# zhan994/agi_lidar_slam

Measured on AMD Instinct MI355X. Metric: IKF iterations/sec, 100k-pt scan vs 10M-pt map, higher is better.
Workload: dtype f32 (kNN, plane) + f64 (Jacobian, reduction, 24x24 update); 1 GPU; C2: S-FAST_LIO update_iterated_dyn_share_modified, 100000-pt Avia scan vs 10000000-pt map, 4 IKF iterations per step with the 5-NN search every iteration; map_points=10000000, scan_points=100000, control_flow=fixed, maximum_iter=4, ikf_loop=device-resident, parallelism=single GPU, effective_points=91373

## Files before the change

### agi_lidar_slam_amd/csrc/slio_device.hip

```cpp
#include <hip/hip_ext.h>
#include <hip/hip_runtime.h>
#include <hipcub/hipcub.hpp>
#include <rccl/rccl.h>

#include <algorithm>
#include <type_traits>
#include <atomic>
#include <cmath>
#include <cstdlib>
#include <cstdio>
#include <cstddef>
#include <cstring>
#include <type_traits>
#include <memory>
#include <mutex>
#include <shared_mutex>
#include <string>
#include <vector>

#include "slio_common.hpp"
#include "slio_cvsolve.hpp"
#include "slio_device.hpp"
#include "slio_frontend.h"
#include "slio_plane.hpp"
// ... 1689 lines not shown
      row[12] = -(double)pd2;
      row[13] = 1.0;
    }
    st_out(out.sel + i, (uint8_t)(sel ? 1 : 0));
  }
  st_out(out.resid + i, sel ? pd2 : __int_as_float(0x7fc00000));
}

__device__ __forceinline__ double chunk_sums_256(double (*rows)[kRow], double (*part)[SLIO_NPROD],
                                                 bool mfma) {
  return mfma ? chunk_products_mfma_v<256>(rows) : chunk_products_v<256>(rows, part);
}

template <bool SC1>
__device__ __forceinline__ void ikf_dx_new(IkfCtl* ctl) {
  if (blockIdx.x != 0) return;
  const int t = threadIdx.x;
  auto ld = [](const double* p) { return SC1 ? ld_sc1(p) : *p; };
  if (t < 24) {
    const int k = t;
    if (k < 3 || k >= 9) {
      const double* xs = reinterpret_cast<const double*>(&ctl->x);
      const double* ps = reinterpret_cast<const double*>(&ctl->xprop);
      st_sc1(&ctl->dxn[k], ld(xs + state_off(k)) - ld(ps + state_off(k)));
    }
  } else if (t == 32 || t == 64) {
    const int u = t == 32;
    const double* q1 = u ? ctl->x.rli : ctl->x.rot;
    const double* q2 = u ? ctl->xprop.rli : ctl->xprop.rot;
    double d[3];
    so3_boxminus(Quat{ld(q1), ld(q1 + 1), ld(q1 + 2), ld(q1 + 3)}, Quat{ld(q2), ld(q2 + 1), ld(q2 + 2), ld(q2 + 3)},
                 d);
    st_sc1(&ctl->dxn[3 + 3 * u], d[0]);
    st_sc1(&ctl->dxn[4 + 3 * u], d[1]);
    st_sc1(&ctl->dxn[5 + 3 * u], d[2]);
  }
}

struct FuseArgs {
  IkfCtl* ctl;
  const IkfCtl* pre;
  double* seg_out;
  double* super_out;
  const IkfCtl* src;
  IkfCtl* hblk;
  uint32_t* cnt;
  double R;
  int iter, maxit;
  int64_t C;
  int nrows, s0, granks;
  double* gsup;
  uint32_t* garrive;
  int32_t gseq;
  uint64_t* goflag;
  uint64_t wait_ticks;
};
constexpr int kGoFlagStride = 16;
constexpr int kSegCnt = 16;
constexpr int kCountWords = kSegCnt + kNSeg;
constexpr int kKcCount = 8;

__device__ __forceinline__ int seg_of_chunk(int64_t C, int64_t c, int64_t& lim) {
  int s = 0;
#pragma unroll
  for (int q = 1; q < SLIO_NSUPER; ++q) s = super_lo(C, q) <= c ? q : s;
  const int64_t c0 = super_lo(C, s), c1 = super_lo(C, s + 1);
  const int g = (int)((c - c0) % kSuperSeg);
  lim = (c1 - c0 - g + kSuperSeg - 1) / kSuperSeg;
  return s * kSuperSeg + g;
}

template <int D>
__device__ __forceinline__ void prefetch_ctl(const IkfCtl* __restrict__ hsrc, IkfCtl* __restrict__ ctl) {
  constexpr int nC = CtlList<D>::total;
  const double* hs = reinterpret_cast<const double*>(hsrc);
  double* cd = reinterpret_cast<double*>(ctl);
  for (int e = threadIdx.x; e < nC; e += blockDim.x) {
    const int o = ctl_src<D>(e);
    st_sc1(cd + o, ld_sys(hs + o));
  }
  if (threadIdx.x < 8)
    st_sc1_u32(reinterpret_cast<uint32_t*>(&ctl->converge) + threadIdx.x,
               ld_sys_u32(reinterpret_cast<const uint32_t*>(&hsrc->converge) + threadIdx.x));
  if (threadIdx.x == 8) st_sc1_u32(reinterpret_cast<uint32_t*>(&ctl->singular), 0u);
  if (threadIdx.x == 9)
    st_sc1_u32(reinterpret_cast<uint32_t*>(&ctl->seq), ld_sys_u32(reinterpret_cast<const uint32_t*>(&hsrc->seq)));
}

template <int NT, int D, bool WT = false>
__device__ __forceinline__ void fused_tail(StepLds& L, int& bcast, const FuseArgs& fa, IkfCtl* ctl,
                                           const double* chunk_part, int64_t chunk, int iter) {
  const int t = threadIdx.x;
  int64_t lim;
  const int b = seg_of_chunk(fa.C, chunk, lim);
#ifdef SLIO_SOLVE_STAMP
  unsigned long long ts[4] = {0, 0, 0, 0};
  if (t == 0) ts[0] = wall_clock64();
#endif
  drain_stores();
  __syncthreads();
  if (t == 0) bcast = (int)arrive(fa.cnt + kSegCnt + b);
  __syncthreads();
#ifdef SLIO_SOLVE_STAMP
  if (t == 0) ts[1] = wall_clock64();
#endif
  if (bcast != (int)lim - 1) return;
  if (t < SLIO_NPROD) {
    const int s = b / kSuperSeg, g = b - s * kSuperSeg;
    const double* p = chunk_part + (super_lo(fa.C, s) + g) * SLIO_NPROD + t;
    constexpr int kJ = 16;
    double acc = 0.0;
    for (int64_t j0 = 0; j0 < lim; j0 += kJ) {
      double v[kJ];
#pragma unroll
      for (int j = 0; j < kJ; ++j) v[j] = (j0 + j < lim) ? ld_sc1(p + (j0 + j) * (kSuperSeg * SLIO_NPROD)) : 0.0;
#pragma unroll
      for (int j = 0; j < kJ; ++j) acc = acc + v[j];
    }
    st_sc1(fa.seg_out + b * SLIO_NPROD + t, acc);
  }
  if (t == 0) reset_counter(fa.cnt + kSegCnt + b);
  drain_stores();
  __syncthreads();
#ifdef SLIO_SOLVE_STAMP
  if (t == 0) ts[2] = wall_clock64();
#endif
  if (t == 0) bcast = (int)arrive(fa.cnt);
  __syncthreads();
  if (bcast != fa.nrows - 1) return;
#ifdef SLIO_SOLVE_STAMP
  if (t == 0) {
    ts[3] = wall_clock64();
    for (int k = 0; k < 4; ++k) g_sstamp[16 + k] = ts[k];
    g_sstamp[36 + ((iter + 1) & 3)] = ts[0];
    g_sstamp[32 + ((iter + 1) & 3)] = ts[3];
  }
#endif
  if (t == 0) {
    reset_counter(fa.cnt);
    st_sc1_u32(fa.cnt + 6, ld_sc1_u32(fa.cnt + 5));
    st_sc1_u32(fa.cnt + 4, 0u);
    st_sc1_u32(fa.cnt + 5, 0u);
  }
  if (!fa.gsup) {
    final_step<NT, D, true, false, WT>(L, fa.seg_out, fa.super_out, ctl, fa.src, fa.hblk, fa.R, iter, fa.maxit);
    if (WT && fa.goflag) {
      drain_stores();
      __syncthreads();
      if (t < 8) {
        const uint64_t fl = ((uint64_t)(uint32_t)fa.gseq << 32) | (L.fl[F_DONE] ? 0x80000000ull : 0ull) |
                            (uint64_t)(uint32_t)L.fl[F_PASSES];
        __hip_atomic_store((guint64*)(fa.goflag + t * kGoFlagStride), fl, __ATOMIC_RELAXED,
                           __HIP_MEMORY_SCOPE_AGENT);
      }
    }
  } else {
    const int nsup = SLIO_NSUPER / fa.granks;
    if (t < SLIO_NPROD) {
      for (int k = 0; k < nsup; ++k) {
        const int ss = fa.s0 + k;
        double a = ld_sc1(fa.seg_out + (ss * kSuperSeg) * SLIO_NPROD + t);
#pragma unroll
        for (int q = 1; q < kSuperSeg; ++q) a = a + ld_sc1(fa.seg_out + (ss * kSuperSeg + q) * SLIO_NPROD + t);
        st_sc1(fa.gsup + ss * SLIO_NPROD + t, a);
      }
      if (!fa.garrive)
        for (int ss = 0; ss < SLIO_NSUPER; ++ss)
          if (ss < fa.s0 || ss >= fa.s0 + nsup) st_sc1(fa.gsup + ss * SLIO_NPROD + t, 0.0);
    }
    if (!fa.garrive) return;
    drain_stores();
    __syncthreads();
    if (t == 0) bcast = (int)arrive(fa.garrive);
    __syncthreads();
    if (bcast != fa.granks - 1) return;
    if (t == 0) reset_counter(fa.garrive);
    final_step<NT, D, true, true>(L, fa.gsup, nullptr, ctl, fa.src, fa.hblk, fa.R, iter, fa.maxit);
    drain_stores();
    __syncthreads();
    if (t == 0) {
      __builtin_amdgcn_fence(__ATOMIC_RELEASE, "agent");
      asm volatile("s_waitcnt vmcnt(0)" ::: "memory");
      const uint64_t fl = ((uint64_t)(uint32_t)fa.gseq << 32) | (L.fl[F_DONE] ? 0x80000000ull : 0ull) |
                          (uint64_t)(uint32_t)L.fl[F_PASSES];
      __hip_atomic_store((guint64*)(uint64_t*)(fa.garrive + 2), fl, __ATOMIC_RELAXED, __HIP_MEMORY_SCOPE_AGENT);
    }
  }
#ifdef SLIO_SOLVE_STAMP
  if (t == 0) g_sstamp[25 + ((iter + 1) & 3)] = wall_clock64();
#endif
}

#ifndef SLIO_RL8_MAX
#define SLIO_RL8_MAX 8
#endif
struct RefLds {
  uint64_t top[SLIO_CHUNK][5];
  float4 q[SLIO_CHUNK];
  uint8_t slot[SLIO_CHUNK];
};
template <int NT>
struct SearchLds {
  union {
    double rows[SLIO_CHUNK][kRow];
    RefLds ref;
  } rr;
  double part[NT / 128][SLIO_NPROD];
  alignas(16) uint32_t nb_pos[SLIO_CHUNK][5];
  alignas(16) float nb_sqd[SLIO_CHUNK][5];
  alignas(16) int32_t nb_idx[SLIO_CHUNK][5];
  float nb_d5[SLIO_CHUNK];
  float4 qw[SLIO_CHUNK];
  float4 qb[SLIO_CHUNK];
  float4 qpl[SLIO_CHUNK];
  uint32_t kc_n[2];
  uint32_t kx6[SLIO_CHUNK];
  uint8_t ksame[SLIO_CHUNK];
  int far_cnt, ref_cnt;
  uint32_t cost;
  uint32_t tab_pre[NT / 16][kTab];
  int32_t tab_dl[NT / 16][kTab];
  float4 far_q[SLIO_CHUNK];
  uint8_t far_slot[SLIO_CHUNK];
  uint32_t far_pre[NT / 64][64], far_beg[NT / 64][64];
};
template <int NT>
union PassLds {
  SearchLds<NT> s;
  StepLds L;
};

template <int LPQ, int U, bool SPHERE, bool DEVPOSE, bool FUSE, int FD, bool PERS>
__device__ __forceinline__ void search_pass_body(PassLds<search_block<LPQ>()>& lds, int& fuse_bcast,
                                                 const MapView& map, const ScanDev& scan, const PoseDev& pose,
                                                 const PassCfg& cfg, const PassOut& out, const FuseArgs& fa,
                                                 bool reuse, int iter) {
  constexpr int NT = search_block<LPQ>();
  constexpr bool KC = DEVPOSE && LPQ == 2 && !SPHERE;
  if (DEVPOSE) ikf_dx_new<PERS>(cfg.ctl);
  constexpr int QPP = NT / LPQ;
  constexpr int PASSES = SLIO_CHUNK / QPP;
  static_assert(SLIO_CHUNK % QPP == 0, "chunk must be a multiple of queries/pass");
  static_assert(NT >= SLIO_CHUNK, "fit phase needs one lane per point");
  auto& rows = lds.s.rr.rows;
  auto& ref = lds.s.rr.ref;
  auto& part = lds.s.part;
  auto& nb_pos = lds.s.nb_pos;
  auto& nb_sqd = lds.s.nb_sqd;
  auto& nb_idx = lds.s.nb_idx;
  auto& nb_d5 = lds.s.nb_d5;
  auto& qw = lds.s.qw;
  auto& far_cnt = lds.s.far_cnt;
  auto& ref_cnt = lds.s.ref_cnt;
  auto& tab_pre = lds.s.tab_pre;
  auto& tab_dl = lds.s.tab_dl;
  auto& far_q = lds.s.far_q;
  auto& far_slot = lds.s.far_slot;
  auto& far_pre = lds.s.far_pre;
  auto& far_beg = lds.s.far_beg;
  int64_t chunk = xcd_chunk(cfg.c_begin, cfg.c_end - cfg.c_begin);
  const int tid = threadIdx.x;
  if (reuse) {
    if (tid < SLIO_CHUNK) {
      double row[kRow];
      reuse_row(scan, pose, cfg, out, chunk * SLIO_CHUNK + tid, row);
#pragma unroll
      for (int j = 0; j < kRow; ++j) lds.s.rr.rows[tid][j] = row[j];
    }
    __syncthreads();
  } else {
  if (cfg.perm) {
    const uint32_t pc = cfg.perm[chunk - cfg.c_begin];
    if (pc < (uint32_t)(cfg.c_end - cfg.c_begin)) chunk = cfg.c_begin + pc;
  }
  const int sub = tid & (LPQ - 1);
  const int grp = tid / LPQ;
  const GridGeom g = map.g;
  const float4* __restrict__ pts = map.pts;
  const uint32_t* __restrict__ start = map.start;
  bool cache_ok = false;
  if constexpr (KC) {
    const uint32_t ke = PERS ? __builtin_amdgcn_readfirstlane(ld_sc1_u32(&out.kepoch[chunk])) : out.kepoch[chunk];
    cache_ok = cfg.kc_epoch != 0 && ke == cfg.kc_epoch;
  }
  if (tid == 0) STAMP(0);
  if (tid == 0) {
    far_cnt = 0;
    ref_cnt = 0;
    lds.s.cost = 0;
    if (KC) lds.s.kc_n[0] = lds.s.kc_n[1] = 0;
    if (blockIdx.x == 0 && !cfg.knn_only) *out.pose = pose;
  }
// ... 407 lines not shown
      }
    }
    FSTAMP(3, false);
#pragma unroll
    for (int j = 0; j < kRow; ++j) rows[slot][j] = row[j];
    FSTAMP(4, true);
  }
  __syncthreads();
  if (tid == 0) STAMP(2);
  if (tid == 0 && out.chunk_cost)
    out.chunk_cost[chunk - cfg.c_begin] = lds.s.cost + 256u * (uint32_t)ref_cnt + 1024u * (uint32_t)nfar;
  if constexpr (KC) {
    if (tid == 0 && cfg.kc_epoch) {
      if (!cache_ok) out.kepoch[chunk] = cfg.kc_epoch;
      if (out.kc_count) {
        atomicAdd(out.kc_count, lds.s.kc_n[0]);
        atomicAdd(out.kc_count + 1, lds.s.kc_n[1]);
      }
    }
  }
  {
    const int64_t base = chunk * SLIO_CHUNK;
    const int nw = (int)(5 * min((int64_t)SLIO_CHUNK, scan.n - base));
    const int na = cfg.knn_only ? 3 : 1;
    auto dst = [&](int a) {
      return a == 0 ? out.nbr_pos + base * 5
                    : (uint32_t*)(a == 1 ? (void*)out.nbr_idx : (void*)out.nbr_sqd) + base * 5;
    };
    auto src = [&](int a) {
      return a == 0 ? &nb_pos[0][0]
                    : (const uint32_t*)(a == 1 ? (const void*)&nb_idx[0][0] : (const void*)&nb_sqd[0][0]);
    };
    if ((nw & 3) == 0) {
      const int nv = nw >> 2;
      for (int k = tid; k < na * nv; k += NT) {
        const int a = k >= nv ? (k >= 2 * nv ? 2 : 1) : 0;
        const int v = k - a * nv;
        st_out(reinterpret_cast<uint4*>(dst(a)) + v, reinterpret_cast<const uint4*>(src(a))[v]);
      }
    } else {
      for (int k = tid; k < na * nw; k += NT) {
        const int a = k >= nw ? (k >= 2 * nw ? 2 : 1) : 0;
        const int v = k - a * nw;
        st_out(dst(a) + v, src(a)[v]);
      }
    }
  }
  }
  if (cfg.knn_only) return;
  if constexpr (FUSE) {
    const double pv = chunk_sums_256(rows, part, cfg.mfma);
    if (tid < SLIO_NPROD) st_sc1(out.chunk_part + chunk * SLIO_NPROD + tid, pv);
    if (tid == 0) STAMP(3);
    fused_tail<NT, FD, PERS>(lds.L, fuse_bcast, fa, fa.ctl, out.chunk_part, chunk, iter);
  } else {
    if constexpr (NT == 256) {
      const double pv = chunk_sums_256(rows, part, cfg.mfma);
      if (tid < SLIO_NPROD) out.chunk_part[chunk * SLIO_NPROD + tid] = pv;
    } else {
      chunk_products<NT>(rows, part, out.chunk_part + chunk * SLIO_NPROD);
    }
    if (tid == 0) STAMP(3);
  }
}

template <int LPQ, int U, bool SPHERE, bool DEVPOSE, bool FUSE = false, int FD = 6>
__global__ __launch_bounds__(search_block<LPQ>(), SPHERE ? 2 : 4) void k_search_pass(
    const MapView map, const ScanDev scan, const PoseDev pose_arg, const PassCfg cfg,
    const PassOut out, const FuseArgs fa) {
  static_assert(!FUSE || search_block<LPQ>() == kSolveThreads, "fused pass: 256 threads");
#ifdef SLIO_SOLVE_STAMP
  if (FUSE && blockIdx.x == 0 && threadIdx.x == 0) {
    g_sstamp[20] = wall_clock64();
    g_sstamp[21 + ((fa.iter + 1) & 3)] = g_sstamp[20];
  }
#endif
  if constexpr (FUSE && !DEVPOSE)
    if (blockIdx.x == 0 && fa.pre) prefetch_ctl<FD>(fa.pre, fa.ctl);
  if (DEVPOSE && (cfg.ctl->done || cfg.ctl->passes != cfg.pass_idx ||
                  (!FUSE && cfg.ctl->search_now != cfg.want_search) || (cfg.seq && cfg.ctl->seq != cfg.seq)))
    return;
  __shared__ PassLds<search_block<LPQ>()> lds;
  __shared__ int fuse_bcast;
  const PoseDev pose = DEVPOSE ? pose_of_ctl(cfg.ctl, cfg.pass_idx) : pose_arg;
  bool reuse = false;
  if constexpr (FUSE && DEVPOSE) reuse = !cfg.ctl->search_now;
  search_pass_body<LPQ, U, SPHERE, DEVPOSE, FUSE, FD, false>(lds, fuse_bcast, map, scan, pose, cfg, out, fa,
                                                            reuse, fa.iter);
}

template <int U, int FD>
__global__ __launch_bounds__(kSolveThreads, 4) void k_update_persist(const MapView map, const ScanDev scan,
                                                                     const PoseDev pose0, const PassCfg cfg,
                                                                     const PassOut out, const FuseArgs fa,
                                                                     const int npasses) {
  __shared__ PassLds<kSolveThreads> lds;
  __shared__ int fuse_bcast;
  __shared__ int s_go;
#ifdef SLIO_SOLVE_STAMP
  if (blockIdx.x == 0 && threadIdx.x == 0) {
    g_sstamp[20] = wall_clock64();
    g_sstamp[21 + ((fa.iter + 1) & 3)] = g_sstamp[20];
  }
#endif
  if (blockIdx.x == 0 && fa.pre) prefetch_ctl<FD>(fa.pre, fa.ctl);
  search_pass_body<2, U, false, false, true, FD, true>(lds, fuse_bcast, map, scan, pose0, cfg, out, fa, false,
                                                       fa.iter);
  const uint64_t* flag = fa.goflag + (blockIdx.x & 7) * kGoFlagStride;
  int p = 1;
  if (npasses < 0) goto run;
wait:
  if (p >= npasses) return;
  if (threadIdx.x == 0) {
    int go = 0;
    const unsigned long long t0 = wall_clock64();
    const unsigned long long lim = fa.wait_ticks ? fa.wait_ticks : 100000000ull;
#ifdef SLIO_SOLVE_STAMP
    if (blockIdx.x == 0) g_sstamp[40 + ((fa.iter + p + 1) & 3)] = t0;
#endif
    while (true) {
      if (lim == 1) {
        __hip_atomic_store(&fa.hblk->timeout, 1, __ATOMIC_RELAXED, __HIP_MEMORY_SCOPE_SYSTEM);
        break;
      }
      const uint64_t fl = __hip_atomic_load((const guint64*)flag, __ATOMIC_RELAXED, __HIP_MEMORY_SCOPE_AGENT);
      if ((int32_t)(fl >> 32) == fa.gseq) {
        if (fl & 0x80000000ull) break;
        if ((int32_t)(fl & 0x7fffffffull) >= p) {
          go = (int)(fl & 0x7fffffffull);
          break;
        }
      }
      if (wall_clock64() - t0 > lim) {
        __hip_atomic_store(&fa.hblk->timeout, 1, __ATOMIC_RELAXED, __HIP_MEMORY_SCOPE_SYSTEM);
        break;
      }
      __builtin_amdgcn_s_sleep(4);
    }
    s_go = go;
#ifdef SLIO_SOLVE_STAMP
    if (blockIdx.x == 0) g_sstamp[21 + ((fa.iter + p + 1) & 3)] = wall_clock64();
// ... 152 lines not shown
#pragma unroll
    for (int u = 0; u < kR; ++u) {
      const int e = t + u * NT;
      rv[u] = e < kNSeg * SLIO_NPROD ? ld_sc1(seg_out + e) : 0.0;
    }
#pragma unroll
    for (int u = 0; u < kR; ++u) {
      const int e = t + u * NT;
      if (e < kNSeg * SLIO_NPROD) (&sh.seg[0][0])[e] = rv[u];
    }
    __syncthreads();
    if (t < SLIO_NPROD) {
#pragma unroll
      for (int ss = 0; ss < SLIO_NSUPER; ++ss) {
        double a = sh.seg[ss * kSuperSeg][t];
#pragma unroll
        for (int q = 1; q < kSuperSeg; ++q) a = a + sh.seg[ss * kSuperSeg + q][t];
        super_out[ss * SLIO_NPROD + t] = a;
      }
    }
  }
}

template <int D>
__global__ __launch_bounds__(kSolveThreads) void k_ikf_solve(IkfCtl* ctl, const IkfCtl* src,
                                                             IkfCtl* hblk, const double* sup,
                                                             double R, int i, int maxit) {
  __shared__ StepLds L;
  step_load<kSolveThreads, D, SLIO_NSUPER * SLIO_NPROD>(L, &L.sup[0][0], sup, false, src, ctl);
  __syncthreads();
  step_totals(L, R);
  __syncthreads();
  if (src == ctl && L.fl[F_DONE]) return;
  ikf_step<kSolveThreads, D>(ctl, hblk, R, i, maxit, L);
}

int dev_users(int device, int delta) {
  static std::atomic<int> users[256];
  if (device < 0 || device >= 256) return 0;
  return users[device].fetch_add(delta) + delta;
}

static bool env_on(const char* name) {
  const char* e = std::getenv(name);
  return e && e[0] && e[0] != '0';
}
static void load_switches(Ctx& c) {
  c.sw.no_fuse = env_on("SLIO_NO_FUSE");
  c.sw.no_fuse0 = env_on("SLIO_NO_FUSE0");
  c.sw.no_mfma = env_on("SLIO_NO_MFMA");
  c.sw.event_wait = env_on("SLIO_EVENT_WAIT");
  c.sw.no_kc = env_on("SLIO_NO_KNN_CERT");
  c.sw.persist = env_on("SLIO_PERSIST");
}
static inline int64_t mono_ns() {
  timespec ts;
  clock_gettime(CLOCK_MONOTONIC, &ts);
  return (int64_t)ts.tv_sec * 1000000000LL + ts.tv_nsec;
}
#define SLIO_HSTAMP(c, k) \
  do {                    \
    if ((c).hstamp) (c).hst[k] = mono_ns(); \
  } while (0)

static std::pair<hipEvent_t, hipEvent_t> prof_pair(Ctx& c) {
  if (!c.pool.empty()) {
    auto p = c.pool.back();
    c.pool.pop_back();
    return p;
  }
  std::pair<hipEvent_t, hipEvent_t> p{nullptr, nullptr};
  (void)hipEventCreate(&p.first);
  (void)hipEventCreate(&p.second);
  return p;
}

static void prof_drain(Ctx& c) {
  for (int k = 0; k < 3; ++k) {
    for (auto& p : c.pending[k]) {
      float ms = 0.f;
      if (hipEventSynchronize(p.second) == hipSuccess &&
          hipEventElapsedTime(&ms, p.first, p.second) == hipSuccess) {
        c.prof_ms[k] += ms;
        c.prof_n[k] += 1;
      }
      c.pool.push_back(p);
    }
    c.pending[k].clear();
  }
}

static int map_write_begin(Ctx& c) {
  MapDev& m = *c.map;
  for (Ctx* u : m.users) {
    if (u == &c || u->stream == c.stream) continue;
    if (!u->map_ev) SLIO_HIP(hipEventCreateWithFlags(&u->map_ev, hipEventDisableTiming));
    SLIO_HIP(hipEventRecord(u->map_ev, u->stream));
    SLIO_HIP(hipStreamWaitEvent(c.stream, u->map_ev, 0));
  }
  if (m.ready && c.seen_epoch != m.epoch) SLIO_HIP(hipStreamWaitEvent(c.stream, m.ready, 0));
  return SLIO_OK;
}
static int map_write_end(Ctx& c) {
  MapDev& m = *c.map;
  if (!m.ready) SLIO_HIP(hipEventCreateWithFlags(&m.ready, hipEventDisableTiming));
  SLIO_HIP(hipEventRecord(m.ready, c.stream));
// ... 252 lines not shown
  cfg.pass_idx = sa ? sa->pass_idx : 0;
  cfg.knn_only = knn_only ? 1 : 0;
  cfg.mfma = !c.sw.no_mfma;
  static const bool no_order = std::getenv("SLIO_NO_CHUNK_ORDER") != nullptr;
  cfg.perm = (devpose && !fuse && c.cus_per_xcd > 0 && !no_order) ? c.chunk_perm : nullptr;
  if (int rc = map_refresh(c); rc) return rc;
  if (which != 0 && c.map->blk_deferred) {
    std::unique_lock<std::shared_mutex> lk(c.map->mu);
    if (c.map->blk_deferred && (c.map->stable_passes += (persist > 0 ? persist : 1)) > kBlkAfterPasses) {
      if (int rc = map_write_begin(c)) return rc;
      if (int rc = build_blk(*c.map, c.stream, "slio map"); rc) return rc;
      if (int rc = map_write_end(c)) return rc;
    }
  }
  std::shared_lock<std::shared_mutex> map_lock(c.map->mu);
  if (int rc = map_read_sync(c)) return rc;
  if (!devpose) c.kc_version = c.map->version;
  cfg.kc_epoch = ((devpose || persist) && c.kq && c.map->version == c.kc_version) ? c.kc_epoch : 0;
  cfg.seq = fuse ? c.group_seq : 0;
  PassOut o{c.nbr_idx,    c.nbr_pos,    c.nbr_sqd,   c.plane,  c.sel,    c.resid,
            c.chunk_part, c.count + 4, c.nbr_pose, c.chunk_cost, c.kq, c.k6,
            c.kepoch,     c.kc_stats ? c.count + kKcCount : nullptr};
  ScanDev s = sd ? *sd : ScanDev{c.bx, c.by, c.bz, c.n};
  const PoseDev P = Parg ? *Parg : PoseDev{};
  const int64_t nblk = c1 - c0;
  if (c.prof && (c.pending[0].size() + c.pending[1].size()) > 256) prof_drain(c);
  const bool run_search = which != 0, run_reuse = which != 1 && !fuse;
  auto timing = [&](int kind) {
    std::pair<hipEvent_t, hipEvent_t> ev{nullptr, nullptr};
    if (c.prof && (c.prof_mask & (1 << kind))) {
      ev = prof_pair(c);
      c.pending[kind].push_back(ev);
    }
    return ev;
  };
  if (nblk > 0 && run_search) {
    const auto ev = timing(SLIO_KERNEL_SEARCH);
    const CoarseView cv{c.map->cg, c.map->clo, c.map->chi};
    const MapView mv{c.map->g,   c.map->n,    c.map->pts,    c.map->start, c.map->blk,
                     c.map->bstart, c.map->nblk, c.map->ncells, cv};
    const bool sph = cfg.radius_sq > 0.0f;
    const dim3 nb((unsigned)nblk);
#define SLIO_LAUNCH(L, SPH, DEV)                                                                   \
  hipExtLaunchKernelGGL(k_search_pass<L, SLIO_SEARCH_U, SPH, DEV>, nb, dim3(search_block<L>()), 0, c.stream, \
                        ev.first, ev.second, 0, mv, s, P, cfg, o, FuseArgs{})
#define SLIO_LAUNCH2(L, SPH) \
  do {                        \
    if (devpose)              \
      SLIO_LAUNCH(L, SPH, true); \
    else                      \
      SLIO_LAUNCH(L, SPH, false); \
  } while (0)
    if (fuse) {
#define SLIO_LAUNCH_FUSED(DEV, D)                                                                           \
  hipExtLaunchKernelGGL(k_search_pass<2, SLIO_SEARCH_U, false, DEV, true, D>, nb, dim3(kSolveThreads), 0, \
                        c.stream, ev.first, ev.second, 0, mv, s, P, cfg, o, *fuse)
#define SLIO_LAUNCH_PERSIST(D)                                                                    \
  hipExtLaunchKernelGGL(k_update_persist<SLIO_SEARCH_U, D>, nb, dim3(kSolveThreads), 0, c.stream, ev.first, \
                        ev.second, 0, mv, s, P, cfg, o, *fuse, persist)
      if (persist > 0) {
        if (sa && sa->dim == 12)
          SLIO_LAUNCH_PERSIST(12);
        else
          SLIO_LAUNCH_PERSIST(6);
      } else if (sa && sa->dim == 12) {
        if (devpose)
          SLIO_LAUNCH_FUSED(true, 12);
        else
          SLIO_LAUNCH_FUSED(false, 12);
      } else {
        if (devpose)
          SLIO_LAUNCH_FUSED(true, 6);
        else
          SLIO_LAUNCH_FUSED(false, 6);
      }
#undef SLIO_LAUNCH_FUSED
#undef SLIO_LAUNCH_PERSIST
    } else
    switch (c.prm.lanes_per_query * 2 + (sph ? 1 : 0)) {
      case 2: SLIO_LAUNCH2(1, false); break;
      case 3: SLIO_LAUNCH2(1, true); break;
      case 8: SLIO_LAUNCH2(4, false); break;
      case 9: SLIO_LAUNCH2(4, true); break;
      case 16: SLIO_LAUNCH2(8, false); break;
      case 17: SLIO_LAUNCH2(8, true); break;
      case 5: SLIO_LAUNCH2(2, true); break;
      default: SLIO_LAUNCH2(2, false); break;
    }
#undef SLIO_LAUNCH2
#undef SLIO_LAUNCH
    c.nbr_lazy = !knn_only;
    c.nbr_stale = false;
  }
  if (nblk > 0 && run_reuse) {
    const auto ev = timing(SLIO_KERNEL_REUSE);
    PassCfg rcfg = cfg;
    rcfg.want_search = 0;
    const dim3 nb((unsigned)nblk), bs(256);
    if (devpose)
      hipExtLaunchKernelGGL(k_reuse_pass<true>, nb, bs, 0, c.stream, ev.first, ev.second, 0, s, P,
                            rcfg, o);
    else
      hipExtLaunchKernelGGL(k_reuse_pass<false>, nb, bs, 0, c.stream, ev.first, ev.second, 0, s, P,
                            rcfg, o);
  }
  if (with_super && !fuse) enqueue_super(c, ctl, sa);
  SLIO_HIP(hipGetLastError());
  if (which != 0) {
    c.searched = true;
    c.search_version = c.map->version;
  }
  return SLIO_OK;
}

static int nbr_settle(Ctx& c) {
  if (!c.nbr_lazy) return SLIO_OK;
  c.nbr_lazy = false;
  if (!c.map || c.search_version != c.map->version) {
    c.nbr_stale = true;
    return SLIO_OK;
  }
  int64_t c0, c1;
  rank_chunks(c.n, c.prm.rank, c.prm.nranks, &c0, &c1);
  const int64_t b = c0 * SLIO_CHUNK, e = std::min(c1 * SLIO_CHUNK, c.n);
  if (e <= b || !c.map) return SLIO_OK;
  k_nbr_derive<<<(unsigned)((e - b + 255) / 256), 256, 0, c.stream>>>(ScanDev{c.bx, c.by, c.bz, c.n}, c.map->pts,
                                                         c.nbr_pos, c.nbr_pose, b, e, c.nbr_idx,
                                                         c.nbr_sqd);
  SLIO_HIP(hipGetLastError());
// ... 3191 lines not shown
    first = (mode == SLIO_MODE_REFERENCE) ? -1 : 0;
    if (++c.kc_next == 0) {
      if (c.kepoch) SLIO_HIP(hipMemsetAsync(c.kepoch, 0, 4 * (num_chunks(c.prm.max_points) + 1), c.stream));
      c.kc_next = 1;
    }
    c.kc_epoch = c.sw.no_kc ? 0 : c.kc_next;
    dim = ext ? 12 : 6;
    slio_pose p;
    std::memcpy(p.rot, x->rot, sizeof(p.rot));
    std::memcpy(p.pos, x->pos, sizeof(p.pos));
    std::memcpy(p.rli, x->rli, sizeof(p.rli));
    std::memcpy(p.tli, x->tli, sizeof(p.tli));
    pose0 = make_pose(&p);
    return SLIO_OK;
  }

  void fill_block() {
    IkfCtl& hc = *c.h_ctl;
    hc.x = *x;
    hc.xprop = *x;
    std::memcpy(hc.P, P, sizeof(double) * 576);
    hc.converge = 1;
    hc.t = 0;
    hc.done = 0;
    hc.search_now = 1;
    hc.passes = hc.searches = hc.valid_passes = 0;
    hc.mode = mode;
    hc.last_m = 0;
    hc.singular = 0;
    hc.published = 0;
    hc.timeout = 0;
    for (int k = 0; k < 24; ++k) hc.dxn[k] = 0.0;
  }

  SolveArgs args(int i) const {
    const bool p0 = i == first;
    const IkfCtl* src = p0 ? (const IkfCtl*)c.d_hctl : c.ctl;
    return SolveArgs{multi ? 0 : 1, dim, i - first, i, maxit, R, src, c.d_hctl};
  }

  int pass(int i) {
    const bool p0 = i == first;
    const SolveArgs sa = args(i);
    const int which = p0 ? 1 : (mode == SLIO_MODE_FIXED ? 1 : 2);
    if (fusable() && !(p0 && c.sw.no_fuse0)) {
      if (p0) {
        fill_block();
        if (!info_constants(P, dim, c.h_ctl->P11i, c.h_ctl->G)) {
          set_error("slio_ikf_update_device: singular covariance block P[:D, :D]");
          return SLIO_EINVAL;
        }
        SLIO_HSTAMP(c, 2);
      }
      const FuseArgs fa{c.ctl,   p0 ? (const IkfCtl*)c.d_hctl : nullptr,
                        c.d_seg, c.d_super,
                        c.ctl,   c.d_hctl,
                        c.count, R,
                        i,       maxit,
                        num_chunks(c.n), kNSeg,
                        0,       1,
                        nullptr, nullptr,
                        0};
      int rc = enqueue_pass(c, p0 ? &pose0 : nullptr, c.ctl, which, ext, &sa, true, false, nullptr, &fa);
      if (rc) return rc;
      if (p0) SLIO_HSTAMP(c, 3);
      SLIO_HIP(hipGetLastError());
      return SLIO_OK;
    }
    if (fused_rows() && !(p0 && c.sw.no_fuse0)) {
      const int nr = c.prm.nranks;
      const FuseArgs fa{c.ctl,   nullptr,
                        c.d_seg, c.d_super,
                        c.ctl,   c.d_hctl,
                        c.count, R,
                        i,       maxit,
                        num_chunks(c.n), kNSeg / nr,
                        c.prm.rank * (SLIO_NSUPER / nr), nr,
                        c.d_super, nullptr,
                        0};
      if (p0) fill_block();
      if (p0 && !info_constants(P, dim, c.h_ctl->P11i, c.h_ctl->G)) {
        set_error("slio_ikf_update_device: singular covariance block P[:D, :D]");
        return SLIO_EINVAL;
      }
      int rc = enqueue_pass(c, p0 ? &pose0 : nullptr, c.ctl, which, ext, &sa, true, false, nullptr, &fa);
      if (rc) return rc;
      SLIO_HIP(hipGetLastError());
      return SLIO_OK;
    }
    int rc = enqueue_pass(c, p0 ? &pose0 : nullptr, c.ctl, which, ext, &sa, !p0 || multi);
    if (rc) return rc;
    if (p0) {
      fill_block();
      if (!info_constants(P, dim, c.h_ctl->P11i, c.h_ctl->G)) {
        (void)hipStreamSynchronize(c.stream);
        set_error("slio_ikf_update_device: singular covariance block P[:D, :D]");
        return SLIO_EINVAL;
      }
      if (!multi) enqueue_super(c, c.ctl, &sa);
    }
    SLIO_HIP(hipGetLastError());
    return SLIO_OK;
  }

  bool fused_ok() const {
    const int lpq = c.prm.lanes_per_query;
    return !c.sw.no_fuse && (lpq != 1 && lpq != 4 && lpq != 8) && !(c.prm.search_radius > 0.0f) &&
           num_chunks(c.n) >= (int64_t)kNSeg;
  }
  bool fusable() const {
    const bool off = c.sw.no_fuse;
    const int lpq = c.prm.lanes_per_query;
    return !off && !multi && c.prm.nranks == 1 &&
           (lpq != 1 && lpq != 4 && lpq != 8) && !(c.prm.search_radius > 0.0f) &&
           num_chunks(c.n) >= (int64_t)kNSeg;
// ... 15 lines not shown
      c.persist_cap = (int64_t)std::min(b6, b12) * c.ncu;
    }
    return num_chunks(c.n) <= c.persist_cap;
  }
  int persist() {
    fill_block();
    if (!info_constants(P, dim, c.h_ctl->P11i, c.h_ctl->G)) {
      set_error("slio_ikf_update_device: singular covariance block P[:D, :D]");
      return SLIO_EINVAL;
    }
    if (++c.upd_seq <= 0) c.upd_seq = 1;
    c.h_ctl->seq = c.upd_seq;
    SLIO_HSTAMP(c, 2);
    const SolveArgs sa = args(first);
    FuseArgs fa{c.ctl,   (const IkfCtl*)c.d_hctl,
                c.d_seg, c.d_super,
                c.ctl,   c.d_hctl,
                c.count, R,
                first,   maxit,
                num_chunks(c.n), kNSeg,
                0,       1,
                nullptr, nullptr,
                c.upd_seq};
    fa.goflag = c.goflag;
    fa.wait_ticks = c.wait_ticks;
    if (int rc = enqueue_pass(c, &pose0, c.ctl, 1, ext, &sa, true, false, nullptr, &fa, maxit - first)) return rc;
    SLIO_HSTAMP(c, 3);
    SLIO_HIP(hipGetLastError());
    return SLIO_OK;
  }

  int solve(int i) {
    const SolveArgs sa = args(i);
    if (dim == 12)
      k_ikf_solve<12><<<1, kSolveThreads, 0, c.stream>>>(c.ctl, sa.src, c.d_hctl, c.d_super, R, i, maxit);
    else
      k_ikf_solve<6><<<1, kSolveThreads, 0, c.stream>>>(c.ctl, sa.src, c.d_hctl, c.d_super, R, i, maxit);
    SLIO_HIP(hipGetLastError());
    return SLIO_OK;
  }

  int finish(slio_ikf_stats* stats) {
    SLIO_HSTAMP(c, 4);
    SLIO_HIP(wait_published(c));
    SLIO_HSTAMP(c, 5);
    const IkfCtl& hc = *c.h_ctl;
    if (!hc.done || hc.timeout) {
      const bool to = hc.timeout != 0;
      const std::string st = "(passes " + std::to_string(hc.passes) + ", searches " + std::to_string(hc.searches) +
                             ", converge " + std::to_string(hc.converge) + ", published " +
                             std::to_string(hc.published) + ")";
      reset_update_counters(c);
      if (to) {
        set_error("slio_ikf_update_device: a device-side wait gave up (persistent pass flag or group gate, "
                  "> 1 s) " + st + "; the handle's arrival counters were reset");
        return SLIO_ETIMEOUT;
      }
      set_error("slio_ikf_update_device: the update did not complete " + st);
      return SLIO_EDEVICE;
    }
    if (hc.singular) {
      set_error("slio_ikf_update_device: singular covariance");
      return SLIO_EINVAL;
    }
    *x = hc.x;
    std::memcpy(P, hc.P, sizeof(double) * 576);
    if (stats) {
      stats->passes = hc.passes;
      stats->searches = hc.searches;
      stats->valid_passes = hc.valid_passes;
      stats->converged = hc.converge;
      stats->last_m = hc.last_m;
      stats->device_ms = 0.0;
    }
    return SLIO_OK;
  }
};

struct GroupSupers {
  double* sup[SLIO_NSUPER];
  int n;
};
__global__ __launch_bounds__(256) void k_group_reduce(GroupSupers g) {
  for (int e = threadIdx.x; e < SLIO_NSUPER * SLIO_NPROD; e += blockDim.x) {
    double v = g.sup[0][e];
    for (int r = 1; r < g.n; ++r) v = v + g.sup[r][e];
    for (int r = 0; r < g.n; ++r) g.sup[r][e] = v;
  }
}

__global__ __launch_bounds__(64) void k_group_gate(const uint32_t* __restrict__ garrive, int pass_idx, int32_t seq,
                                                   IkfCtl* __restrict__ hblk, uint64_t wait_ticks) {
  if (threadIdx.x != 0) return;
  const unsigned long long t0 = wall_clock64();
  const unsigned long long lim = wait_ticks ? wait_ticks : 100000000ull;
  if (lim == 1) {
    __hip_atomic_store(&hblk->timeout, 1, __ATOMIC_RELAXED, __HIP_MEMORY_SCOPE_SYSTEM);
    return;
  }
  while (true) {
    const uint64_t fl = __hip_atomic_load((const guint64*)(const uint64_t*)(garrive + 2), __ATOMIC_RELAXED,
                                          __HIP_MEMORY_SCOPE_AGENT);
    const int32_t fseq = (int32_t)(fl >> 32);
    const bool done = (fl & 0x80000000ull) != 0;
    const int32_t passes = (int32_t)(fl & 0x7fffffffull);
    if ((fseq == seq && (done || passes >= pass_idx)) || (int32_t)(fseq - seq) > 0) return;
    if (wall_clock64() - t0 > lim) {
// ... 189 lines not shown
                        int extrinsic_est, int mode, slio_ikf_stats* stats) {
  const int kind = hs[0]->c.group_reduce;
  std::vector<slio_state> xs((size_t)n, *x);
  std::vector<std::vector<double>> Ps((size_t)n, std::vector<double>(P, P + 576));
  std::vector<UpdateRun> runs;
  runs.reserve((size_t)n);
  for (int r = 0; r < n; ++r)
    runs.emplace_back(hs[r]->c, &xs[r], Ps[r].data(), R, maximum_iter, extrinsic_est, mode, true);
  for (int r = 0; r < n; ++r) {
    SLIO_HIP(hipSetDevice(hs[r]->c.prm.device));
    if (int rc = runs[r].begin()) return rc;
  }
  GroupSupers gs{};
  gs.n = n;
  for (int r = 0; r < n; ++r) gs.sup[r] = hs[r]->c.d_super;
  Ctx& c0 = hs[0]->c;
  bool gfused = kind == 2 && c0.gsup && n > 1 && runs[0].fused_ok();
  for (int r = 1; r < n && gfused; ++r) gfused = hs[r]->c.prm.device == c0.prm.device;
  if (gfused) {
    const int64_t C = num_chunks(c0.n);
    const bool hs_on = c0.hstamp;
    if (hs_on) {
      c0.hst[0] = mono_ns();
      c0.hst[4] = c0.hst[5] = c0.hst[6] = 0;
    }
    if (++c0.upd_seq <= 0) c0.upd_seq = 1;
    const int32_t seq = c0.upd_seq;
    for (int r = 0; r < n; ++r) hs[r]->c.group_seq = seq;
    int rc = SLIO_OK;
    for (int i = runs[0].first; i < maximum_iter && !rc; ++i) {
      const bool p0 = i == runs[0].first;
      if (p0) {
        runs[0].fill_block();
        c0.h_ctl->seq = seq;
        if (!info_constants(P, runs[0].dim, c0.h_ctl->P11i, c0.h_ctl->G)) {
          set_error("slio_group_ikf_update: singular covariance block P[:D, :D]");
          rc = SLIO_EINVAL;
          break;
        }
      }
      const int which = p0 ? 1 : (mode == SLIO_MODE_FIXED ? 1 : 2);
      for (int r = 0; r < n && !rc; ++r) {
        Ctx& cr = hs[r]->c;
        if (!p0) k_group_gate<<<1, 64, 0, cr.stream>>>(c0.garrive, i - runs[0].first, seq, c0.d_hctl, c0.wait_ticks);
        const SolveArgs sa = runs[r].args(i);
        const FuseArgs fa{c0.ctl,  (p0 && r == 0) ? (const IkfCtl*)c0.d_hctl : nullptr,
                          cr.d_seg, c0.gsup,
                          c0.ctl,  c0.d_hctl,
                          cr.count, R,
                          i,       maximum_iter,
                          C,       kNSeg / n,
                          r * (SLIO_NSUPER / n), n,
                          c0.gsup, c0.garrive,
                          seq,     nullptr,
                          c0.wait_ticks};
        rc = enqueue_pass(cr, p0 ? &runs[r].pose0 : nullptr, c0.ctl, which, extrinsic_est, &sa, true, false,
                          nullptr, &fa);
        if (!rc && hipGetLastError() != hipSuccess) {
          set_error("slio_group_ikf_update: launch failed");
          rc = SLIO_EDEVICE;
        }
      }
    }
    for (int r = 0; r < n; ++r) hs[r]->c.group_seq = 0;
    if (rc) return rc;
    if (hs_on) {
      c0.hst[1] = mono_ns();
      c0.hst[4] = c0.hst[1] - c0.hst[0];
    }
    {
      volatile int32_t* pub = &c0.h_ctl->published;
      for (uint32_t it = 1; !*pub; ++it) {
        if ((it & 255) == 0) {
          bool idle = true;
          for (int r = 0; r < n && idle; ++r) {
            const hipError_t e = hipStreamQuery(hs[r]->c.stream);
            if (e != hipSuccess && e != hipErrorNotReady) return SLIO_EDEVICE;
            idle = e == hipSuccess;
          }
          if (idle) break;
        }
        __builtin_ia32_pause();
      }
      std::atomic_thread_fence(std::memory_order_acquire);
    }
    if (hs_on) c0.hst[2] = mono_ns();
    slio_ikf_stats st0{};
    c0.hstamp = false;
    const int rc2 = runs[0].finish(&st0);
    c0.hstamp = hs_on;
    if (rc2) return rc2;
    *x = xs[0];
    std::memcpy(P, Ps[0].data(), sizeof(double) * 576);
    if (stats) *stats = st0;
    if (hs_on) c0.hst[3] = mono_ns();
    return SLIO_OK;
  }
  const bool hs_on = c0.hstamp;
  int64_t t_a = 0;
  if (hs_on) {
    c0.hst[0] = mono_ns();
    c0.hst[4] = c0.hst[5] = c0.hst[6] = 0;
  }
  for (int i = runs[0].first; i < maximum_iter; ++i) {
    if (hs_on) t_a = mono_ns();
    for (int r = 0; r < n; ++r) {
      SLIO_HIP(hipSetDevice(hs[r]->c.prm.device));
      if (int rc = runs[r].pass(i)) return rc;
// ... 231 lines not shown
```

### agi_lidar_slam_amd/csrc/slio_device.hpp

```cpp
#pragma once

#include <hip/hip_runtime.h>

#include <algorithm>
#include <atomic>
#include <cstdint>
#include <memory>
#include <shared_mutex>
#include <string>
#include <utility>
#include <vector>

#include "slio_common.hpp"
#include "slio_search.hpp"

#define SLIO_HIP(call)                                                          \
  do {                                                                          \
    hipError_t e_ = (call);                                                     \
    if (e_ != hipSuccess) {                                                     \
      set_error(std::string(#call) + ": " + hipGetErrorString(e_));             \
      return SLIO_EDEVICE;                                                      \
    }                                                                           \
  } while (0)

// ... 123 lines not shown
  double* chunk_part = nullptr;
  uint32_t* chunk_cost = nullptr;
  float4* kq = nullptr;
  uint32_t* k6 = nullptr;
  uint32_t* kepoch = nullptr;
  uint32_t kc_next = 0;
  uint32_t kc_epoch = 0;
  uint64_t kc_version = 0;
  bool kc_stats = false;
  uint32_t* chunk_perm = nullptr;
  int cus_per_xcd = 0;
  double* d_super = nullptr;
  double* d_super_own = nullptr;
  double* d_seg = nullptr;
  void* comm = nullptr;
  int group_reduce = 0;
  hipEvent_t grp_ev = nullptr;
  double* gsup = nullptr;
  uint32_t* garrive = nullptr;
  int32_t group_seq = 0;
  int32_t upd_seq = 0;
  uint32_t* count = nullptr;
  MapDev::Buf inc[7];
  MapDev::Buf pre[16];
  float* kfx = nullptr;
  float* kfy = nullptr;
  float* kfz = nullptr;
  int64_t kf_used = 0, kf_cap = 0;
  std::vector<int64_t> kf_off, kf_len;
  MapDev::Buf kfb[3];
  hipEvent_t kf_ev = nullptr;
  MapDev::Buf icp[5];
  int64_t icp_n = -1;
  int64_t icp_far = 0;
  IkfCtl* ctl = nullptr;
  IkfCtl* h_ctl = nullptr;
  IkfCtl* d_hctl = nullptr;
  hipEvent_t done_ev = nullptr;
  double* h_super = nullptr;
  bool searched = false;
  bool prof = false;
  int prof_mask = 0;
  std::vector<std::pair<hipEvent_t, hipEvent_t>> pending[3];
  std::vector<std::pair<hipEvent_t, hipEvent_t>> pool;
  double prof_ms[3] = {0, 0, 0};
  int64_t prof_n[3] = {0, 0, 0};
  struct Switches {
    bool no_fuse = false;
    bool no_fuse0 = false;
    bool no_mfma = false;
    bool event_wait = false;
    bool no_kc = false;
    bool persist = false;
  } sw;
  uint64_t* goflag = nullptr;
  int ncu = 0;
  int64_t persist_cap = -1;
  int last_path = 0;
  bool dev_counted = false;
  uint64_t wait_ticks = 0;
  bool hstamp = false;
  int64_t hst[8] = {};
};

struct Rb {
  void* dst;
  const void* src;
  size_t n;
};

struct KfSeg {
  const float *x, *y, *z;
  uint32_t off;
  uint32_t pad;
  float m[12];
};
constexpr int kKfTile = 256;

struct LegoRot {
  float cr, sr, cp, sp, cy, sy, tx, ty, tz;
};
__device__ __forceinline__ void lego_to_map(const LegoRot& T, float x, float y, float z, float& ox, float& oy,
                                            float& oz) {
  const float x1 = T.cy * x - T.sy * y;
  const float y1 = T.sy * x + T.cy * y;
  const float z1 = z;
  const float x2 = x1;
  const float y2 = T.cr * y1 - T.sr * z1;
  const float z2 = T.sr * y1 + T.cr * z1;
  ox = T.cp * x2 + T.sp * z2 + T.tx;
  oy = y2 + T.ty;
  oz = -T.sp * x2 + T.cp * z2 + T.tz;
}

struct SolveArgs;
struct FuseArgs;

#pragma GCC visibility push(hidden)
int map_read_sync(Ctx& c);
PoseDev make_pose(const slio_pose* x);
hipError_t readback(hipStream_t st, const Rb* rb, int k);
int map_refresh(Ctx& c, bool adds_only = false);
int enqueue_pass(Ctx& c, const PoseDev* Parg, IkfCtl* ctl, int which, int extrinsic_est,
                 const SolveArgs* sa = nullptr, bool with_super = true, bool knn_only = false,
                 const ScanDev* sd = nullptr, const FuseArgs* fuse = nullptr, int persist = 0);
int grid_blocks(int64_t n);
// ... 22 lines not shown
```

Baseline: 29360 IKF iterations/s.

## Add dedicated reducer workgroup that polls segment-ready flags and runs the IKF step

The fused search pass gets one extra workgroup that, instead of the last-arriving block doing the segment and global reductions via counter chains, spins on per-segment ready flags. It loads each finished segment row as soon as it appears, sums the super-segments in registers, and runs the IKF step. The aim is to take the serialized second-level arrive/reduce tail off the critical path and overlap the final reduction with the remaining search blocks. The cost is one workgroup held spinning through the whole pass, which could deadlock or time out if the grid does not fit on the device. A watchdog timeout and an environment switch to disable the reducer are included.

```diff
diff --git a/agi_lidar_slam_amd/csrc/slio_device.hip b/agi_lidar_slam_amd/csrc/slio_device.hip
--- a/agi_lidar_slam_amd/csrc/slio_device.hip
+++ b/agi_lidar_slam_amd/csrc/slio_device.hip
@@ -1765,11 +1765,13 @@
   double* gsup;
   uint32_t* garrive;
   int32_t gseq;
+  int32_t reducer;
   uint64_t* goflag;
   uint64_t wait_ticks;
 };
 constexpr int kGoFlagStride = 16;
 constexpr int kSegCnt = 16;
+constexpr uint32_t kRowReady = 0x80000000u;
 constexpr int kCountWords = kSegCnt + kNSeg;
 constexpr int kKcCount = 8;
 
@@ -1800,7 +1802,7 @@
     st_sc1_u32(reinterpret_cast<uint32_t*>(&ctl->seq), ld_sys_u32(reinterpret_cast<const uint32_t*>(&hsrc->seq)));
 }
 
-template <int NT, int D, bool WT = false>
+template <int NT, int D, bool WT = false, bool RED = false>
 __device__ __forceinline__ void fused_tail(StepLds& L, int& bcast, const FuseArgs& fa, IkfCtl* ctl,
                                            const double* chunk_part, int64_t chunk, int iter) {
   const int t = threadIdx.x;
@@ -1832,6 +1834,19 @@
     }
     st_sc1(fa.seg_out + b * SLIO_NPROD + t, acc);
   }
+  if constexpr (RED) {
+    drain_stores();
+    __syncthreads();
+    if (t == 0) st_sc1_u32(fa.cnt + kSegCnt + b, kRowReady);
+#ifdef SLIO_SOLVE_STAMP
+    if (t == 0) {
+      ts[2] = wall_clock64();
+      for (int k = 0; k < 3; ++k)
+        __hip_atomic_fetch_max(&g_sstamp[16 + k], ts[k], __ATOMIC_RELAXED, __HIP_MEMORY_SCOPE_AGENT);
+    }
+#endif
+    return;
+  }
   if (t == 0) reset_counter(fa.cnt + kSegCnt + b);
   drain_stores();
   __syncthreads();
@@ -1902,6 +1917,187 @@
 #ifdef SLIO_SOLVE_STAMP
   if (t == 0) g_sstamp[25 + ((iter + 1) & 3)] = wall_clock64();
 #endif
+}
+
+struct ReducerLds {
+  StepLds L;
+  int stop;
+};
+template <int NT, int D, bool DEVPOSE>
+__device__ __forceinline__ void reducer_pass(ReducerLds& rl, const FuseArgs& fa, int iter) {
+  static_assert(NT == 256 && kNSeg == 64 && SLIO_NPROD <= 128, "reducer: 2 x 128 threads hold 32 rows each");
+  StepLds& L = rl.L;
+  IkfCtl* ctl = fa.ctl;
+  const int t = threadIdx.x;
+#ifdef SLIO_SOLVE_STAMP
+  if (t == 0) g_sstamp[44] = wall_clock64();
+  if (t < 3) __hip_atomic_store(&g_sstamp[16 + t], 0ull, __ATOMIC_RELAXED, __HIP_MEMORY_SCOPE_AGENT);
+#endif
+  const unsigned long long lim = fa.wait_ticks ? fa.wait_ticks : 100000000ull;
+  if (lim == 1) {
+    if (t == 0) {
+      __hip_atomic_store(&fa.hblk->timeout, 1, __ATOMIC_RELAXED, __HIP_MEMORY_SCOPE_SYSTEM);
+      st_sc1_u32(reinterpret_cast<uint32_t*>(&ctl->done), 1u);
+    }
+    return;
+  }
+  const unsigned long long t0 = wall_clock64();
+  {
+    constexpr int nC = CtlList<D>::total, kC = (nC + NT - 1) / NT;
+    const bool first = fa.pre != nullptr;
+    const double* src = reinterpret_cast<const double*>(first ? fa.pre : (const IkfCtl*)ctl);
+    const uint32_t* fsrc = reinterpret_cast<const uint32_t*>(first ? &fa.pre->converge : &ctl->converge);
+    double cv[kC];
+#pragma unroll
+    for (int u = 0; u < kC; ++u) {
+      const int e = t + u * NT;
+      cv[u] = e < nC ? (first ? ld_sys(src + ctl_src<D>(e)) : ld_sc1(src + ctl_src<D>(e))) : 0.0;
+    }
+    uint32_t fl = 0, seq = 0;
+    if (t < 8) fl = first ? ld_sys_u32(fsrc + t) : ld_sc1_u32(fsrc + t);
+    if (first && t == 9) seq = ld_sys_u32(reinterpret_cast<const uint32_t*>(&fa.pre->seq));
+#pragma unroll
+    for (int u = 0; u < kC; ++u) {
+      const int e = t + u * NT;
+      if (e < nC) {
+        ctl_dst<D>(L, e) = cv[u];
+        if (first) st_sc1(reinterpret_cast<double*>(ctl) + ctl_src<D>(e), cv[u]);
+      }
+    }
+    if (t < 8) {
+      L.fl[t] = (int32_t)fl;
+      if (first) st_sc1_u32(reinterpret_cast<uint32_t*>(&ctl->converge) + t, fl);
+    }
+    if (first && t == 8) st_sc1_u32(reinterpret_cast<uint32_t*>(&ctl->singular), 0u);
+    if (first && t == 9) st_sc1_u32(reinterpret_cast<uint32_t*>(&ctl->seq), seq);
+    if (t == 0) rl.stop = 0;
+  }
+  __syncthreads();
+  if constexpr (DEVPOSE) {
+    if (t < 24) {
+      if (t < 3 || t >= 9) {
+        const double* xs = reinterpret_cast<const double*>(&L.x);
+        const double* ps = reinterpret_cast<const double*>(&L.xprop);
+        const double v = xs[state_off(t)] - ps[state_off(t)];
+        L.dxn[t] = v;
+        st_sc1(&ctl->dxn[t], v);
+      }
+    } else if (t == 32 || t == 64) {
+      const int u = t == 32;
+      const double* q1 = u ? L.x.rli : L.x.rot;
+      const double* q2 = u ? L.xprop.rli : L.xprop.rot;
+      double d[3];
+      so3_boxminus(Quat{q1[0], q1[1], q1[2], q1[3]}, Quat{q2[0], q2[1], q2[2], q2[3]}, d);
+#pragma unroll
+      for (int j = 0; j < 3; ++j) {
+        L.dxn[3 + 3 * u + j] = d[j];
+        st_sc1(&ctl->dxn[3 + 3 * u + j], d[j]);
+      }
+    }
+  }
+#ifdef SLIO_SOLVE_STAMP
+  if (t == 0) g_sstamp[45] = wall_clock64();
+#endif
+  const int half = t >> 7, k = t & 127;
+  const bool holder = k < SLIO_NPROD;
+  constexpr int kAnchor[3] = {5, 16, 27};
+  const char* anchor[3];
+#pragma unroll
+  for (int q = 0; q < 3; ++q) {
+    anchor[q] = reinterpret_cast<const char*>(fa.seg_out + (size_t)(32 * half + kAnchor[q]) * SLIO_NPROD +
+                                              (holder ? k : 0));
+    asm volatile("" : "+v"(anchor[q]));
+  }
+  double r[32];
+#pragma unroll
+  for (int j = 0; j < 32; ++j) r[j] = 0.0;
+  const uint32_t* cw = fa.cnt + kSegCnt + (t & 63);
+  const int hsh = 32 * __builtin_amdgcn_readfirstlane(half);
+  unsigned long long seen = 0;
+  auto take = [&](uint32_t c) {
+    const unsigned long long m = __ballot(c == kRowReady) & ~seen;
+    seen |= m;
+    const uint32_t mh = (uint32_t)(m >> hsh);
+#pragma unroll
+    for (int j = 0; j < 32; ++j)
+      if ((mh >> j) & 1u) {
+        constexpr int kRowBytes = SLIO_NPROD * (int)sizeof(double);
+        const int q = j < 11 ? 0 : (j < 22 ? 1 : 2);
+        static_assert(11 * kRowBytes / 2 < 4096, "reducer: rows within a load's immediate offset of an anchor");
+        r[j] = ld_sc1(reinterpret_cast<const double*>(anchor[q] + (j - kAnchor[q]) * kRowBytes));
+      }
+  };
+  bool gave_up = false;
+  uint32_t ca = ld_sc1_u32(cw), cb;
+  for (uint32_t round = 1;; ++round) {
+    cb = ld_sc1_u32(cw);
+    take(ca);
+    if (seen == ~0ull) break;
+    ca = ld_sc1_u32(cw);
+    take(cb);
+    if (seen == ~0ull) break;
+    if ((round & 255u) == 0 && wall_clock64() - t0 > lim) {
+      gave_up = true;
+      break;
+    }
+  }
+#ifdef SLIO_SOLVE_STAMP
+  if (t == 0) g_sstamp[46] = g_sstamp[32 + ((iter + 1) & 3)] = wall_clock64();
+#endif
+  if (gave_up && (t & 63) == 0) rl.stop = 1;
+  double a = 0.0;
+  double sp[4] = {0.0, 0.0, 0.0, 0.0};
+  if (holder) {
+#pragma unroll
+    for (int s = 0; s < 4; ++s) {
+      double v = r[s * kSuperSeg];
+#pragma unroll
+      for (int q = 1; q < kSuperSeg; ++q) v = v + r[s * kSuperSeg + q];
+      sp[s] = v;
+    }
+#ifdef SLIO_SOLVE_STAMP
+    if (t == 0) g_sstamp[47] = wall_clock64();
+#endif
+    if (half) {
+#pragma unroll
+      for (int s = 0; s < 4; ++s) L.sup[4 + s][k] = sp[s];
+    } else {
+      a = ((sp[0] + sp[1]) + sp[2]) + sp[3];
+    }
+  }
+  __syncthreads();
+  if (rl.stop) {
+    if (t == 0) {
+      __hip_atomic_store(&fa.hblk->timeout, 1, __ATOMIC_RELAXED, __HIP_MEMORY_SCOPE_SYSTEM);
+      st_sc1_u32(reinterpret_cast<uint32_t*>(&ctl->done), 1u);
+    }
+    return;
+  }
+  if (t < 64) reset_counter(fa.cnt + kSegCnt + t);
+  if (holder) {
+#pragma unroll
+    for (int s = 0; s < 4; ++s) fa.super_out[(4 * half + s) * SLIO_NPROD + k] = sp[s];
+  }
+  if (holder && !half) {
+#pragma unroll
+    for (int s = 4; s < SLIO_NSUPER; ++s) a = a + L.sup[s][k];
+    L.tot[k] = a;
+    if (k < SLIO_NHTH)
+      L.Mt[k] = a / fa.R;
+    else if (k < SLIO_NHTH + 12)
+      L.hR[k - SLIO_NHTH] = a / fa.R;
+  }
+  __syncthreads();
+  SSTAMP(4);
+  if (!L.fl[F_DONE]) ikf_step<NT, D, false>(ctl, fa.hblk, fa.R, iter, fa.maxit, L);
+  if (t == 0) {
+    st_sc1_u32(fa.cnt + 6, ld_sc1_u32(fa.cnt + 5));
+    st_sc1_u32(fa.cnt + 4, 0u);
+    st_sc1_u32(fa.cnt + 5, 0u);
+#ifdef SLIO_SOLVE_STAMP
+    g_sstamp[25 + ((iter + 1) & 3)] = wall_clock64();
+#endif
+  }
 }
 
 #ifndef SLIO_RL8_MAX
@@ -1941,16 +2137,18 @@
 union PassLds {
   SearchLds<NT> s;
   StepLds L;
+  ReducerLds r;
 };
-
-template <int LPQ, int U, bool SPHERE, bool DEVPOSE, bool FUSE, int FD, bool PERS>
+static_assert(sizeof(ReducerLds) <= sizeof(SearchLds<kSolveThreads>), "the reducer adds no LDS to a pass");
+
+template <int LPQ, int U, bool SPHERE, bool DEVPOSE, bool FUSE, int FD, bool PERS, bool RED = false>
 __device__ __forceinline__ void search_pass_body(PassLds<search_block<LPQ>()>& lds, int& fuse_bcast,
                                                  const MapView& map, const ScanDev& scan, const PoseDev& pose,
                                                  const PassCfg& cfg, const PassOut& out, const FuseArgs& fa,
                                                  bool reuse, int iter) {
   constexpr int NT = search_block<LPQ>();
   constexpr bool KC = DEVPOSE && LPQ == 2 && !SPHERE;
-  if (DEVPOSE) ikf_dx_new<PERS>(cfg.ctl);
+  if (DEVPOSE && !RED) ikf_dx_new<PERS>(cfg.ctl);
   constexpr int QPP = NT / LPQ;
   constexpr int PASSES = SLIO_CHUNK / QPP;
   static_assert(SLIO_CHUNK % QPP == 0, "chunk must be a multiple of queries/pass");
@@ -2464,7 +2662,7 @@
     const double pv = chunk_sums_256(rows, part, cfg.mfma);
     if (tid < SLIO_NPROD) st_sc1(out.chunk_part + chunk * SLIO_NPROD + tid, pv);
     if (tid == 0) STAMP(3);
-    fused_tail<NT, FD, PERS>(lds.L, fuse_bcast, fa, fa.ctl, out.chunk_part, chunk, iter);
+    fused_tail<NT, FD, PERS, RED>(lds.L, fuse_bcast, fa, fa.ctl, out.chunk_part, chunk, iter);
   } else {
     if constexpr (NT == 256) {
       const double pv = chunk_sums_256(rows, part, cfg.mfma);
@@ -2476,11 +2674,12 @@
   }
 }
 
-template <int LPQ, int U, bool SPHERE, bool DEVPOSE, bool FUSE = false, int FD = 6>
+template <int LPQ, int U, bool SPHERE, bool DEVPOSE, bool FUSE = false, int FD = 6, bool RED = false>
 __global__ __launch_bounds__(search_block<LPQ>(), SPHERE ? 2 : 4) void k_search_pass(
     const MapView map, const ScanDev scan, const PoseDev pose_arg, const PassCfg cfg,
     const PassOut out, const FuseArgs fa) {
   static_assert(!FUSE || search_block<LPQ>() == kSolveThreads, "fused pass: 256 threads");
+  static_assert(!RED || FUSE, "a reducer workgroup: fused single-rank passes only");
 #ifdef SLIO_SOLVE_STAMP
   if (FUSE && blockIdx.x == 0 && threadIdx.x == 0) {
     g_sstamp[20] = wall_clock64();
@@ -2488,17 +2687,23 @@
   }
 #endif
   if constexpr (FUSE && !DEVPOSE)
-    if (blockIdx.x == 0 && fa.pre) prefetch_ctl<FD>(fa.pre, fa.ctl);
+    if (!RED && blockIdx.x == 0 && fa.pre) prefetch_ctl<FD>(fa.pre, fa.ctl);
   if (DEVPOSE && (cfg.ctl->done || cfg.ctl->passes != cfg.pass_idx ||
                   (!FUSE && cfg.ctl->search_now != cfg.want_search) || (cfg.seq && cfg.ctl->seq != cfg.seq)))
     return;
   __shared__ PassLds<search_block<LPQ>()> lds;
   __shared__ int fuse_bcast;
+  if constexpr (RED) {
+    if ((int64_t)blockIdx.x == cfg.c_end - cfg.c_begin) {
+      reducer_pass<kSolveThreads, FD, DEVPOSE>(lds.r, fa, fa.iter);
+      return;
+    }
+  }
   const PoseDev pose = DEVPOSE ? pose_of_ctl(cfg.ctl, cfg.pass_idx) : pose_arg;
   bool reuse = false;
   if constexpr (FUSE && DEVPOSE) reuse = !cfg.ctl->search_now;
-  search_pass_body<LPQ, U, SPHERE, DEVPOSE, FUSE, FD, false>(lds, fuse_bcast, map, scan, pose, cfg, out, fa,
-                                                            reuse, fa.iter);
+  search_pass_body<LPQ, U, SPHERE, DEVPOSE, FUSE, FD, false, RED>(lds, fuse_bcast, map, scan, pose, cfg, out,
+                                                                 fa, reuse, fa.iter);
 }
 
 template <int U, int FD>
@@ -2757,6 +2962,7 @@
   c.sw.event_wait = env_on("SLIO_EVENT_WAIT");
   c.sw.no_kc = env_on("SLIO_NO_KNN_CERT");
   c.sw.persist = env_on("SLIO_PERSIST");
+  c.sw.no_reducer = env_on("SLIO_NO_REDUCER");
 }
 static inline int64_t mono_ns() {
   timespec ts;
@@ -3115,9 +3321,17 @@
       SLIO_LAUNCH(L, SPH, false); \
   } while (0)
     if (fuse) {
-#define SLIO_LAUNCH_FUSED(DEV, D)                                                                           \
-  hipExtLaunchKernelGGL(k_search_pass<2, SLIO_SEARCH_U, false, DEV, true, D>, nb, dim3(kSolveThreads), 0, \
-                        c.stream, ev.first, ev.second, 0, mv, s, P, cfg, o, *fuse)
+#define SLIO_LAUNCH_FUSED_R(DEV, D, RED)                                                               \
+  hipExtLaunchKernelGGL(k_search_pass<2, SLIO_SEARCH_U, false, DEV, true, D, RED>,                       \
+                        dim3((unsigned)nblk + (RED ? 1u : 0u)), dim3(kSolveThreads), 0, c.stream, ev.first, \
+                        ev.second, 0, mv, s, P, cfg, o, *fuse)
+#define SLIO_LAUNCH_FUSED(DEV, D)         \
+  do {                                    \
+    if (fuse->reducer)                    \
+      SLIO_LAUNCH_FUSED_R(DEV, D, true);  \
+    else                                  \
+      SLIO_LAUNCH_FUSED_R(DEV, D, false); \
+  } while (0)
 #define SLIO_LAUNCH_PERSIST(D)                                                                    \
   hipExtLaunchKernelGGL(k_update_persist<SLIO_SEARCH_U, D>, nb, dim3(kSolveThreads), 0, c.stream, ev.first, \
                         ev.second, 0, mv, s, P, cfg, o, *fuse, persist)
@@ -3138,6 +3352,7 @@
           SLIO_LAUNCH_FUSED(false, 6);
       }
 #undef SLIO_LAUNCH_FUSED
+#undef SLIO_LAUNCH_FUSED_R
 #undef SLIO_LAUNCH_PERSIST
     } else
     switch (c.prm.lanes_per_query * 2 + (sph ? 1 : 0)) {
@@ -6435,15 +6650,17 @@
         }
         SLIO_HSTAMP(c, 2);
       }
-      const FuseArgs fa{c.ctl,   p0 ? (const IkfCtl*)c.d_hctl : nullptr,
-                        c.d_seg, c.d_super,
-                        c.ctl,   c.d_hctl,
-                        c.count, R,
-                        i,       maxit,
-                        num_chunks(c.n), kNSeg,
-                        0,       1,
-                        nullptr, nullptr,
-                        0};
+      FuseArgs fa{c.ctl,   p0 ? (const IkfCtl*)c.d_hctl : nullptr,
+                  c.d_seg, c.d_super,
+                  c.ctl,   c.d_hctl,
+                  c.count, R,
+                  i,       maxit,
+                  num_chunks(c.n), kNSeg,
+                  0,       1,
+                  nullptr, nullptr,
+                  0};
+      fa.reducer = c.sw.no_reducer ? 0 : 1;
+      fa.wait_ticks = c.wait_ticks;
       int rc = enqueue_pass(c, p0 ? &pose0 : nullptr, c.ctl, which, ext, &sa, true, false, nullptr, &fa);
       if (rc) return rc;
       if (p0) SLIO_HSTAMP(c, 3);
@@ -6565,7 +6782,7 @@
                              std::to_string(hc.published) + ")";
       reset_update_counters(c);
       if (to) {
-        set_error("slio_ikf_update_device: a device-side wait gave up (persistent pass flag or group gate, "
+        set_error("slio_ikf_update_device: a device-side wait gave up (reducer rows, persistent pass flag or group gate, "
                   "> 1 s) " + st + "; the handle's arrival counters were reset");
         return SLIO_ETIMEOUT;
       }
@@ -6861,8 +7078,8 @@
                           C,       kNSeg / n,
                           r * (SLIO_NSUPER / n), n,
                           c0.gsup, c0.garrive,
-                          seq,     nullptr,
-                          c0.wait_ticks};
+                          seq,     0,
+                          nullptr, c0.wait_ticks};
         rc = enqueue_pass(cr, p0 ? &runs[r].pose0 : nullptr, c0.ctl, which, extrinsic_est, &sa, true, false,
                           nullptr, &fa);
         if (!rc && hipGetLastError() != hipSuccess) {
diff --git a/agi_lidar_slam_amd/csrc/slio_device.hpp b/agi_lidar_slam_amd/csrc/slio_device.hpp
--- a/agi_lidar_slam_amd/csrc/slio_device.hpp
+++ b/agi_lidar_slam_amd/csrc/slio_device.hpp
@@ -199,6 +199,7 @@
     bool event_wait = false;
     bool no_kc = false;
     bool persist = false;
+    bool no_reducer = false;
   } sw;
   uint64_t* goflag = nullptr;
   int ncu = 0;
```

Result: faster. 30130 IKF iterations/s (median of 6 runs) (+2.6%).
